# hyunlord/hnm_recommendation

Measured on AMD Instinct MI355X. Metric: recommendations/sec (batched users, K=12) at 1/2/4/8 MI355X; % HBM roofline, higher is better.
Workload: dtype f16+f32; 1 GPU; ncf: BASELINE configs[1] NeuralCF dim=64, full H&M shape, batch=4096 users/rank, K=12; users=1371980, items=105542, batch_per_rank=4096, k=12, parallelism=single, model=NeuralCF, mf_dim=64, weights=init, scan=certified f16 pre-filter + exact fp32 re-scoring (ncf_cert.hip)

## Files before the change

hnm_recommendation_amd/_lib.py:

```python
from __future__ import annotations

import ctypes as C
import os
import threading
import weakref

import torch

PKG = os.path.dirname(os.path.abspath(__file__))
LIB_PATH = os.environ.get("HNM_LIB_PATH") or os.path.join(PKG, "libhnm_mi355x.so")

HNM_OK, HNM_EINVAL, HNM_EOOB, HNM_EHIP, HNM_ENOMEM, HNM_EUNSUPPORTED, HNM_ECOLL = 0, -1, -2, -3, -4, -5, -6

_p = C.c_void_p
_i64 = C.c_int64
_i32 = C.c_int32
_f32 = C.c_float


class NcfWeights(C.Structure):
    _fields_ = [("gmf_user", _p), ("gmf_item", _p), ("mlp_user", _p), ("mlp_item", _p),
                ("w1", _p), ("b1", _p), ("w2", _p), ("b2", _p), ("wp", _p), ("bp", _p),
                ("num_users", _i64), ("num_items", _i64), ("mf", _i32), ("h0", _i32),
                ("h1", _i32), ("h2", _i32), ("item_proj", _p)]
# ... 258 lines not shown


def abort_pending(device):
    check(fn("hnm_ctx_abort_pending")(ctx(device)), "hnm_ctx_abort_pending")


def sync_check(device):
    check(fn("hnm_ctx_check")(ctx(device)), "hnm_ctx_check")


TIME_SCORE, TIME_SPMM = 1, 2


def enable_timing(device, on=True):
    check(fn("hnm_ctx_enable_timing")(ctx(device), int(on)), "hnm_ctx_enable_timing")


def kernel_timing(device):
    t = C.c_double()
    n = _i64()
    check(fn("hnm_ctx_timing")(ctx(device), C.byref(t), C.byref(n)), "hnm_ctx_timing")
    return t.value, n.value


HNM_OPT_PREFILTER = 1
HNM_OPT_STATS = 3
HNM_OPT_STRIDED = 4
HNM_OPT_DEEP_MFMA = 5
HNM_OPT_LINEAR_MFMA = 6
HNM_OPT_NCF_TABLES = 7
HNM_OPT_SCAN_SHAPE = 8
HNM_OPT_SCAN_PIPE = 9
HNM_OPT_SCAN_SPARSE = 10


def set_option(device, option, value):
    idx = _dev_index(device)
    ctx(device)
    with _lock:
        _opts.setdefault(idx, {})[int(option)] = int(value)
    for c in _device_ctxs(idx):
        check(fn("hnm_ctx_set_option")(c.handle, int(option), int(value)), "hnm_ctx_set_option")


def set_prefilter(device, on=True):
    set_option(device, HNM_OPT_PREFILTER, int(bool(on)))


def prefilter_stats(device, reset=False, extended=False):
    ctx(device)
    n = (6 if extended == "gate" else 4) if extended else 3
    tot = [0] * n
    for c in _device_ctxs(_dev_index(device)):
        out = (_i64 * n)()
        check(fn("hnm_ctx_prefilter_stats_ex")(c.handle, out, n, int(reset)),
              "hnm_ctx_prefilter_stats_ex")
        for j in range(n):
            tot[j] += int(out[j])
    return tuple(tot)


def ptr(t):
    return None if t is None else _p(t.data_ptr())
```

hnm_recommendation_amd/csrc/api.hip:

```cpp
#include <stdlib.h>
#include <string.h>

#include "hnm_device.h"
#include "hnm_internal.h"
#include "linear_mfma.h"

static thread_local char g_err[512] = "";

void hnm_set_error(const char* fmt, ...) {
  va_list ap;
  va_start(ap, fmt);
  vsnprintf(g_err, sizeof(g_err), fmt, ap);
  va_end(ap);
}

extern "C" int hnm_abi_version(void) { return HNM_ABI_VERSION; }
extern "C" const char* hnm_last_error(void) { return g_err; }

extern "C" hnm_status hnm_ctx_create(int device, hnm_ctx** out) {
  HNM_REQUIRE(out, HNM_EINVAL, "hnm_ctx_create: out is NULL");
  int ndev = 0;
  HNM_HIP_CHECK(hipGetDeviceCount(&ndev));
  HNM_REQUIRE(device >= 0 && device < ndev, HNM_EINVAL, "hnm_ctx_create: no device %d (%d visible)",
              device, ndev);
  const HnmDeviceGuard guard(device);
  hnm_ctx* c = (hnm_ctx*)calloc(1, sizeof(hnm_ctx));
  HNM_REQUIRE(c, HNM_ENOMEM, "hnm_ctx_create: out of host memory");
  c->device = device;
  c->stream = 0;
  hipDeviceProp_t prop;
  if (hipGetDeviceProperties(&prop, device) == hipSuccess) c->num_cus = prop.multiProcessorCount;
  if (c->num_cus <= 0) c->num_cus = 256;
  c->prefilter = 1;
  c->strided = 0;
  c->deep_mfma = 1;
#ifndef HNM_LINEAR_MFMA_DEFAULT
#define HNM_LINEAR_MFMA_DEFAULT 1
#endif
  c->linear_mfma = HNM_LINEAR_MFMA_DEFAULT;
  c->ncf_tables = 1;
  c->scan_shape = 1;
  c->scan_pipe = 1;
  c->scan_sparse = 1;
  if (hipMalloc((void**)&c->err_dev, 64) != hipSuccess) {
    free(c);
    hnm_set_error("hnm_ctx_create: hipMalloc of the error word failed");
    return HNM_ENOMEM;
  }
  HNM_HIP_CHECK(hipMemset(c->err_dev, 0, 64));
  HNM_HIP_CHECK(hipEventCreateWithFlags(&c->chain_ev, hipEventDisableTiming));
  HNM_HIP_CHECK(hipStreamCreateWithFlags(&c->side, hipStreamNonBlocking));
  HNM_HIP_CHECK(hipEventCreateWithFlags(&c->side_in, hipEventDisableTiming));
  HNM_HIP_CHECK(hipEventCreateWithFlags(&c->side_out, hipEventDisableTiming));
  c->stats_dev = reinterpret_cast<unsigned long long*>(reinterpret_cast<char*>(c->err_dev) + 8);
  *out = c;
  return HNM_OK;
}

extern "C" hnm_status hnm_ctx_destroy(hnm_ctx* ctx) {
  HNM_CTX_DEVICE(ctx);
  if (!ctx) return HNM_OK;
  (void)hipDeviceSynchronize();
  for (int i = 0; i < ctx->cap; ++i) {
    (void)hipEventDestroy(ctx->ev0[i]);
    (void)hipEventDestroy(ctx->ev1[i]);
  }
  free(ctx->ev0);
  free(ctx->ev1);
  hnm_rccl_release(ctx);
  if (ctx->ws) (void)hipFree(ctx->ws);
  if (ctx->err_dev) (void)hipFree(ctx->err_dev);
  (void)hipEventDestroy(ctx->chain_ev);
  (void)hipEventDestroy(ctx->side_in);
  (void)hipEventDestroy(ctx->side_out);
  (void)hipStreamDestroy(ctx->side);
  free(ctx);
// ... 18 lines not shown
  return HNM_OK;
}

extern "C" hnm_status hnm_ctx_set_option(hnm_ctx* ctx, int option, int64_t value) {
  HNM_CTX_DEVICE(ctx);
  HNM_REQUIRE(ctx, HNM_EINVAL, "ctx is NULL");
  switch (option) {
    case HNM_OPT_PREFILTER:
      ctx->prefilter = value != 0;
      return HNM_OK;
    case HNM_OPT_STATS:
      ctx->stats_on = value != 0;
      return HNM_OK;
    case HNM_OPT_STRIDED:
      ctx->strided = value != 0;
      return HNM_OK;
    case HNM_OPT_DEEP_MFMA:
      ctx->deep_mfma = value != 0;
      return HNM_OK;
    case HNM_OPT_LINEAR_MFMA:
      ctx->linear_mfma = value != 0;
      return HNM_OK;
    case HNM_OPT_NCF_TABLES:
      ctx->ncf_tables = value != 0;
      return HNM_OK;
    case HNM_OPT_SCAN_SHAPE:
      ctx->scan_shape = value != 0;
      return HNM_OK;
    case HNM_OPT_SCAN_PIPE:
      ctx->scan_pipe = value != 0;
      return HNM_OK;
    case HNM_OPT_SCAN_SPARSE:
      ctx->scan_sparse = value != 0;
      return HNM_OK;
    default:
      hnm_set_error("hnm_ctx_set_option: unknown option %d", option);
      return HNM_EINVAL;
  }
}

extern "C" hnm_status hnm_ctx_prefilter_stats(hnm_ctx* ctx, int64_t* out, int reset) {
  HNM_CTX_DEVICE(ctx);
  return hnm_ctx_prefilter_stats_ex(ctx, out, 3, reset);
}

extern "C" hnm_status hnm_ctx_prefilter_stats_ex(hnm_ctx* ctx, int64_t* out, int n, int reset) {
  HNM_CTX_DEVICE(ctx);
  HNM_REQUIRE(ctx && out, HNM_EINVAL, "ctx/out is NULL");
  HNM_REQUIRE(n >= 1 && n <= HNM_STATS_N, HNM_EINVAL, "prefilter_stats: 1 <= n <= %d", HNM_STATS_N);
  int prev = -1;
  HNM_HIP_CHECK(hipGetDevice(&prev));
  struct Restore {
    int dev;
    ~Restore() { (void)hipSetDevice(dev); }
  } restore{prev};
  HNM_HIP_CHECK(hipSetDevice(ctx->device));
  HNM_HIP_CHECK(hipDeviceSynchronize());
  unsigned long long v[HNM_STATS_N];
  HNM_HIP_CHECK(hipMemcpy(v, ctx->stats_dev, sizeof(v), hipMemcpyDeviceToHost));
  for (int i = 0; i < n; ++i) out[i] = (int64_t)v[i];
  if (reset) HNM_HIP_CHECK(hipMemset(ctx->stats_dev, 0, sizeof(v)));
  return HNM_OK;
}

extern "C" hnm_status hnm_ctx_num_cus(hnm_ctx* ctx, int* out) {
  HNM_CTX_DEVICE(ctx);
// ... 759 lines not shown
```

hnm_recommendation_amd/csrc/hnm_internal.h:

```cpp
#pragma once
#include <hip/hip_runtime.h>
#include <stdarg.h>
#include <stdint.h>
#include <stdio.h>

#include <algorithm>

#include "../../include/hnm.h"

struct hnm_ctx {
  int device;
  hipStream_t stream;
  hipEvent_t chain_ev;
  hipStream_t side;
  hipEvent_t side_in, side_out;
  void* ws;
  size_t ws_size;
  unsigned* err_dev;
  int num_cus;
  int timing;
  int nev;
  int cap;
  hipEvent_t* ev0;
  hipEvent_t* ev1;
  int prefilter;
  int strided;
  int deep_mfma;
  int linear_mfma;
  int ncf_tables;
  int scan_shape;
  int scan_pipe;
  int scan_sparse;
  void* comm;
  int comm_owned;
  unsigned long long* stats_dev;
  int stats_on;
  struct {
    int kind;
    int64_t B, I;
    int K;
    const void* ids;
    const void* items;
    int flags;
  } pend;
};
struct HnmDeviceGuard {
  int prev = -1;
  explicit HnmDeviceGuard(int device) {
    int cur = -1;
    if (device >= 0 && hipGetDevice(&cur) == hipSuccess && cur != device &&
        hipSetDevice(device) == hipSuccess)
      prev = cur;
  }
  ~HnmDeviceGuard() {
    if (prev >= 0) (void)hipSetDevice(prev);
  }
  HnmDeviceGuard(const HnmDeviceGuard&) = delete;
  HnmDeviceGuard& operator=(const HnmDeviceGuard&) = delete;
};
#define HNM_CTX_DEVICE(c) const HnmDeviceGuard hnm_device_guard_((c) ? (c)->device : -1)
#define HNM_STATS_N 6
#define HNM_PEND_NCF_CERT 1
#define HNM_PEND_NCF_EXACT 2
#define HNM_PEND_DOT_CERT 3
#define HNM_PEND_DOT_EXACT 4
// ... 108 lines not shown
```

hnm_recommendation_amd/csrc/ncf.hip:

```cpp
#include <algorithm>

#include "hnm_device.h"
#include "ncf_internal.h"

template <bool DENSE>
__global__ __launch_bounds__(256, 2) void ncf32_kernel(
    const float* __restrict__ Pu,
    const float* __restrict__ WGu,
    const float* __restrict__ Qi,
    const float* __restrict__ Gi, int64_t ldg, int mf,
    const float* __restrict__ W2, int h1, int h2, const float* __restrict__ b2,
    const float* __restrict__ wm, const float* __restrict__ bp, int64_t B, int64_t I,
    int64_t ipp, const int64_t* __restrict__ mptr, const int32_t* __restrict__ midx, int K,
    float* __restrict__ cand_v, int32_t* __restrict__ cand_i, int NP,
    float* __restrict__ dense, int64_t ldo, const int32_t* __restrict__ rows,
    const int32_t* __restrict__ nrows, int dyn_cus) {
  constexpr int KS = 32;
  constexpr int RS = 68;
  constexpr int NU = 128;
  __shared__ __attribute__((aligned(16))) float qs[TILE * RS];
  __shared__ __attribute__((aligned(16))) float gs[TILE * RS];
  __shared__ __attribute__((aligned(16))) float ps[NU * 64];
  __shared__ __attribute__((aligned(16))) float gsm[4 * 32 * 32];
  extern __shared__ __attribute__((aligned(16))) float lists[];

  const int tid = threadIdx.x, lane = tid & 63, wave = tid >> 6, h = lane >> 5, j = lane & 31;
  int64_t ublk = (int64_t)blockIdx.x * NU;
  int p = blockIdx.y;
  if (rows) B = *nrows;
  if (rows && dyn_cus > 0) {
    const int64_t nb = hnm_cdiv(B, NU);
    const Partition dp = choose_partition(I, nb, dyn_cus);
    NP = dp.np;
    ipp = dp.ipp;
    const int64_t w = blockIdx.x;
    if (w >= nb * NP) return;
    ublk = w / NP * NU;
    p = (int)(w % NP);
  }
  if (ublk >= B || p >= NP) return;
  auto R = [&](int64_t b) -> int64_t { return rows ? (int64_t)rows[b] : b; };
  const int64_t u0 = ublk + wave * 32;
  const int nu = (int)std::max<int64_t>(0, std::min<int64_t>(32, B - u0));
  const int64_t part_start = (int64_t)p * ipp;
  const int64_t part_end = std::min<int64_t>(I, part_start + ipp);
  float* lv_s = lists + wave * 32 * K;
  int* li_s = reinterpret_cast<int*>(lists + 4 * 32 * K) + wave * 32 * K;

  for (int e = tid; e < NU * 16; e += 256) {
// ... 148 lines not shown
          if ((bits >> j) & 1u) score = -__builtin_inff();
        }
        if (DENSE) {
          if (ivalid) dense[(u0 + u) * ldo + item] = score;
        } else {
          const float thv = hnm_readlane_f(tvv, u);
          const int thi = hnm_readlane_i(tvi, u);
          uint64_t m = __ballot(ivalid && (score > thv || (score == thv && (int)item < thi)));
          if (m) {
            float lv = lane < K ? lv_s[u * K + lane] : -__builtin_inff();
            int li = lane < K ? li_s[u * K + lane] : HNM_SENTINEL_IDX;
            while (m) {
              const int l = __builtin_ctzll(m);
              m &= m - 1;
              list1_insert(lv, li, hnm_readlane_f(score, l), (int)base + l, K);
            }
            if (lane < K) { lv_s[u * K + lane] = lv; li_s[u * K + lane] = li; }
            const float nv = hnm_readlane_f(lv, K - 1);
            const int ni = hnm_readlane_i(li, K - 1);
            if (lane == u) { tvv = nv; tvi = ni; }
          }
        }
      }
    }
  }
  if (!DENSE) {
    for (int e = lane; e < nu * K; e += 64) {
      const int u = e / K, s = e % K;
      const int64_t o = ((u0 + u) * NP + p) * K + s;
      cand_v[o] = lv_s[e];
      cand_i[o] = li_s[e] == HNM_SENTINEL_IDX ? -1 : li_s[e];
    }
  }
}

template <int WU, int H1P, int MFH, bool DENSE>
__global__ __launch_bounds__(256, 2) void ncf_generic_kernel(
    const float* __restrict__ Pu,
    const float* __restrict__ WGu,
    const float* __restrict__ Qi,
    const float* __restrict__ Gi, int64_t ldg,
    const float* __restrict__ W2, int h1, int h2, const float* __restrict__ b2,
    const float* __restrict__ wm, const float* __restrict__ bp, int64_t B, int64_t I,
    int64_t ipp, const int64_t* __restrict__ mptr, const int32_t* __restrict__ midx, int K,
    float* __restrict__ cand_v, int32_t* __restrict__ cand_i, int NP,
    float* __restrict__ dense, int64_t ldo) {
  constexpr int KS = H1P / 2;
  constexpr int GW = 2 * MFH;
  constexpr int QRS = H1P + 4;
  constexpr int GRS = GW + 4;
  constexpr int NU = 4 * WU;
  constexpr int QF4 = TILE * H1P / 4 / 256;
  constexpr int GF4 = TILE * GW / 4 / 256;
  static_assert(QF4 >= 1 && GF4 >= 1, "tile too small");
  __shared__ __attribute__((aligned(16))) float qs[2][TILE * QRS];
  __shared__ __attribute__((aligned(16))) float gs[2][TILE * GRS];
  __shared__ __attribute__((aligned(16))) float ps[NU * H1P];
  __shared__ __attribute__((aligned(16))) float ws[NU * GW];
  __shared__ __attribute__((aligned(16))) float2 bw[32];

  const int tid = threadIdx.x;
  const int lane = tid & 63;
  const int wave = tid >> 6;
  const int h = lane >> 5;
  const int j = lane & 31;
  const int64_t ublk = (int64_t)blockIdx.x * NU;
// ... 262 lines not shown
  return HNM_OK;
}

template <bool DENSE>
static void launch_ncf32(hnm_ctx* ctx, dim3 grid, const NcfTabs& t, const hnm_ncf_weights* w,
                         int64_t B, int64_t ipp, const int64_t* mptr, const int32_t* midx, int K,
                         float* cv, int32_t* ci, int NP, float* dense, int64_t ldo,
                         const int32_t* rows = nullptr, const int32_t* nrows = nullptr,
                         int dyn_cus = 0) {
  const size_t lds = DENSE ? 0 : (size_t)4 * 32 * K * 8;
  hipLaunchKernelGGL((ncf32_kernel<DENSE>), grid, dim3(256), lds, ctx->stream, t.Pu, t.WGu, t.Qi,
                     t.G, t.ldg, w->mf, w->w2, w->h1, w->h2, w->b2, w->wp + w->mf, w->bp, B,
                     w->num_items, ipp, mptr, midx, K, cv, ci, NP, dense, ldo, rows, nrows,
                     dyn_cus);
}

template <int WU, int H1P, int MFH, bool DENSE>
static void launch_ncf(hnm_ctx* ctx, dim3 grid, const NcfTabs& t, const hnm_ncf_weights* w,
                       int64_t B, int64_t ipp, const int64_t* mptr, const int32_t* midx, int K,
                       float* cv, int32_t* ci, int NP, float* dense, int64_t ldo) {
  hipLaunchKernelGGL((ncf_generic_kernel<WU, H1P, MFH, DENSE>), grid, dim3(256), 0, ctx->stream,
                     t.Pu, t.WGu, t.Qi, t.G, t.ldg, w->w2, w->h1, w->h2, w->b2, w->wp + w->mf,
                     w->bp, B, w->num_items, ipp, mptr, midx, K, cv, ci, NP, dense, ldo);
}

size_t ncf_list_bytes(int64_t B, int64_t I, int K, int num_cus) {
  const Partition part = choose_partition(I, hnm_cdiv(B, 128), num_cus);
  const int64_t slots = std::max<int64_t>(B * part.np, list_rows_slots(B, I, num_cus));
  return hnm_align((size_t)slots * K * 4);
}

hnm_status ncf_list_rows(hnm_ctx* ctx, const hnm_ncf_weights* w, const NcfTabs& t, int64_t B,
                         const int64_t* mptr, const int32_t* midx, int K, const int32_t* rows,
                         const int32_t* nrows, float* cv, int32_t* ci, float* ov, int64_t* oi) {
  const int64_t grid = list_rows_grid(B, w->num_items, ctx->num_cus);
  launch_ncf32<false>(ctx, dim3((unsigned)grid, 1), t, w, B, 0, mptr, midx, K, cv, ci, 1, nullptr,
                      0, rows, nrows, ctx->num_cus);
  HNM_LAUNCH_CHECK();
  return hnm_topk_merge_rows(ctx, cv, ci, B, 1, 0, K, K, K, ov, oi, rows, nrows, w->num_items,
                             ctx->num_cus);
}

struct NcfCall {
  NcfTabs t;
  bool big;
  void* extra;
};

struct NcfCertUse {
  int K;
  bool strided;
};

static hnm_status ncf_tables(hnm_ctx* ctx, const hnm_ncf_weights* w, const int64_t* ids,
                             int64_t B, size_t extra, NcfCall* out, bool fill = true,
                             const NcfCertUse* cert = nullptr) {
  const bool big = w->h1 > 64 || w->mf > 64;
  const int H1P = big ? 128 : 64, GW = big ? 128 : 64;
  const int64_t I = w->num_items;
  const bool gcopy = (big ? w->mf != GW : w->mf % 4 != 0) || ((uintptr_t)w->gmf_item % 16 != 0);
  const bool qcache = w->item_proj != nullptr;
  const size_t szP = hnm_align((size_t)B * H1P * 4), szW = hnm_align((size_t)B * GW * 4);
  const size_t szQ = qcache ? 0 : hnm_align((size_t)I * H1P * 4);
  const size_t szG = gcopy ? hnm_align((size_t)I * GW * 4) : 0;
  void* wsp = ctx->ws;
  hnm_status st = HNM_OK;
  if (fill) {
    st = hnm_workspace(ctx, szP + szW + szQ + szG + extra, &wsp);
// ... 307 lines not shown
```

hnm_recommendation_amd/csrc/ncf_cert.hip:

```cpp
#include <algorithm>

#include "ncf_cert_internal.h"
#include "sample_kth.h"

namespace {

__device__ __forceinline__ float cert_row_bound(const CertParams* prm, float unit,
                                                const float* Au, int64_t b) {
  return unit * (prm->rho * (prm->c0 + Au[b]) + prm->absb);
}
__device__ __forceinline__ float cert_lower_bound(const CertParams* prm, float unit, float kv,
                                                  float e, const float* bp) {
  float l = (kv - e) / unit + bp[0];
  l -= fabsf(l) * 4.76837158203125e-07f;
  return (!prm->bad && __builtin_isfinite(l) && __builtin_isfinite(e)) ? l : -__builtin_inff();
}

__device__ __forceinline__ void cert_threshold(const CertParams* prm, float unit, const float* Au,
                                               const float* Cu, int64_t b, float l, float e,
                                               const float* bp, float* tau, int* flag) {
  const float scale = unit * (prm->c0 + Au[b] + prm->Bmax + Cu[b] * prm->Dmax);
  float tv = (l - bp[0]) * unit - e - 3.814697265625e-06f * scale;
  tv -= fabsf(tv) * 9.5367431640625e-07f;
  const bool ok = !prm->bad && __builtin_isfinite(tv) && __builtin_isfinite(scale);
// ... 345 lines not shown
  auto take = [&](size_t bytes) {
    char* p = base ? base + off : nullptr;
    off += hnm_align(bytes);
    return p;
  };
  CertWs x;
  x.prm = (CertParams*)take(sizeof(CertParams));
  x.Au = (float*)take(B * 4);
  x.Cu = (float*)take(B * 4);
  x.Cs = (float*)take(B * 4);
  x.Bs = (float*)take(I * 4);
  x.part = (float*)take(4 * 4 * (1024 + 256));
  x.Bi = (float*)take(I * 4);
  x.Di = (float*)take(I * 4);
  x.tau = (float*)take(B * 4);
  x.Eu = (float*)take(B * 4);
  x.b2s = (float*)take(32 * 4);
  x.kthv = (float*)take((size_t)B * K * 4);
  x.lb = (float*)take((size_t)B * 4);
  x.pdense = (float*)take((size_t)CERT_PROXY_USERS * I * 4);
  x.cdense = (float*)take((size_t)B * sh.nch * 4);
  x.sidx = (int32_t*)take((size_t)sh.nch * 4);
  x.sloo = strided ? (int32_t*)take((size_t)CERT_PROXY_USERS * sh.nch * 4) : nullptr;
  x.sidx2 = strided ? (int32_t*)take((size_t)sh.ns * 4) : nullptr;
  x.sdense = strided ? (float*)take((size_t)B * sh.ns * 4) : nullptr;
  x.kth2 = strided ? (float*)take((size_t)B * K * 4) : nullptr;
  x.gate = (int*)take(4);
  x.gcnt = (unsigned long long*)take(4 * 8);
  x.kthi = (int64_t*)take((size_t)B * K * 8);
  x.cnt = (int*)take((size_t)B * sh.part.np * 4);
  x.flag = (int*)take(B * 4);
  x.ovf_cnt = (int32_t*)take(256);
  x.ovf_rows = (int32_t*)take(B * 4);
  x.buf = (int32_t*)take((size_t)B * sh.part.np * sh.capp * 4);
  x.bufd = (float*)take((size_t)B * sh.part.np * sh.capp * 4);
  x.P16 = (_Float16*)take((size_t)B * 64 * 2);
  x.WG16 = (_Float16*)take((size_t)B * 64 * 2);
  x.Q16 = (_Float16*)take((size_t)I * 64 * 2);
  x.G16 = (_Float16*)take((size_t)I * 64 * 2);
  x.W2h = (_Float16*)take(32 * 64 * 2);
  x.wmh = (_Float16*)take(32 * 2);
  x.W3h = (_Float16*)take(16 * 32 * 2);
  x.wph = (_Float16*)take(16 * 2);
  x.b3s = (float*)take(16 * 4);
  x.u = (float*)take(32 * 4);
  const size_t lb = ncf_list_bytes(B, I, K, num_cus);
  x.cv = (float*)take(lb);
  x.ci = (int32_t*)take(lb);
  if (w) *w = x;
  return off;
}

ScanArgs scan_args(const CertWs& x, int64_t B, bool deep) {
  ScanArgs a{};
  a.W3h = deep ? x.W3h : nullptr;
  a.wph = x.wph;
  a.b3s = x.b3s;
  a.P16 = x.P16;
  a.WG16 = x.WG16;
  a.Q16 = x.Q16;
  a.G16 = x.G16;
  a.W2h = x.W2h;
  a.wmh = x.wmh;
  a.b2s = x.b2s;
  a.Bi = x.Bs;
  a.Di = x.Di;
// ... 119 lines not shown
  const CertPlan pl = cert_plan(ctx, B, I, K, scratch, strided);
  const CertShape& sh = pl.sh;
  const CertWs& x = pl.ws;
  const int64_t ublocks = hnm_cdiv(B, 128);
  if (lb != nullptr || strided) {
    hipLaunchKernelGGL(cert_tau_kernel, dim3((unsigned)hnm_cdiv(B, 256)), dim3(256), 0,
                       ctx->stream, lb ? lb : x.lb, x.Au, x.Cu, x.Eu, x.prm, w->bp, B, x.tau,
                       x.flag);
    HNM_LAUNCH_CHECK();
  }
  ScanArgs a = scan_args(x, B, dp != nullptr);
  a.I = I;
  a.mptr = mptr;
  a.midx = midx;
  a.tau = x.tau;
  a.cnt = x.cnt;
  a.buf = x.buf;
  a.segd = x.bufd;
  a.capp = sh.capp;
  a.ipp = sh.part.ipp;
  a.NP = sh.part.np;
  hnm_timer_begin(ctx, HNM_TIME_SCORE);
  cert_launch_scan(ctx, SCAN_THRESH, dim3((unsigned)sh.part.np, (unsigned)ublocks), a);
  hnm_timer_end(ctx, HNM_TIME_SCORE);
  HNM_LAUNCH_CHECK();
  cert_launch_rescore(ctx, w, t, B, pl, K, short_ok, ov, oi, dp);
  HNM_LAUNCH_CHECK();
  if (dp) {
    *ovf_rows = x.ovf_rows;
    *ovf_cnt = x.ovf_cnt;
    return HNM_OK;
  }
  hnm_status st =
      ncf_list_rows(ctx, w, t, B, mptr, midx, K, x.ovf_rows, x.ovf_cnt, x.cv, x.ci, ov, oi);
  if (st || !short_ok) return st;
  return hnm_topk_trim_below(ctx, ov, oi, B, K, lb);
}

hnm_status ncf_cert_topk(hnm_ctx* ctx, const hnm_ncf_weights* w, const NcfTabs& t, int64_t B,
                         const int64_t* mptr, const int32_t* midx, int K, void* scratch,
                         bool strided, float* ov, int64_t* oi) {
  hnm_status st = ncf_cert_begin(ctx, w, t, B, mptr, midx, K, scratch, strided, nullptr);
  if (st) return st;
  return ncf_cert_finish(ctx, w, t, B, mptr, midx, K, scratch, strided, nullptr, 0, ov, oi);
}

hnm_status ncf_deep_cert_topk(hnm_ctx* ctx, const hnm_ncf_weights* w, const CertDeep& dp,
                              const NcfTabs& t, int64_t B, const int64_t* mptr,
                              const int32_t* midx, int K, void* scratch, float* ov, int64_t* oi,
                              int32_t** ovf_rows, int32_t** ovf_cnt, bool* pruned) {
  hnm_status st = ncf_cert_begin(ctx, w, t, B, mptr, midx, K, scratch, false, nullptr, nullptr, &dp);
  if (st) return st;
  const int64_t I = w->num_items;
  const CertPlan pl = cert_plan(ctx, B, I, K, scratch, false);
  const CertShape& sh = pl.sh;
  const CertWs& x = pl.ws;
  const int np_rows = (int)std::min<int64_t>(CERT_PROXY_USERS, B);
  HNM_HIP_CHECK(hipMemsetAsync(x.gcnt, 0, 8, ctx->stream));
  hipLaunchKernelGGL(cert_predict_kernel,
                     dim3((unsigned)std::min<int64_t>(64, hnm_cdiv(I, 256)), (unsigned)np_rows),
                     dim3(256), 0, ctx->stream, x.pdense, I, K, x.kthv, x.Eu, x.Bs, x.Cs, x.Di,
                     x.prm, x.gcnt);
  HNM_LAUNCH_CHECK();
  unsigned long long pc = 0;
  HNM_HIP_CHECK(hipMemcpyAsync(&pc, x.gcnt, 8, hipMemcpyDeviceToHost, ctx->stream));
  HNM_HIP_CHECK(hipStreamSynchronize(ctx->stream));
  const int64_t limit = std::min<int64_t>(I / 16, (int64_t)sh.part.np * sh.capp / 2);
// ... 33 lines not shown
```

hnm_recommendation_amd/csrc/ncf_cert_internal.h:

```cpp
#pragma once
#include "hnm_device.h"
#include "ncf_internal.h"

constexpr int64_t CERT_MIN_ITEMS = 8192;
constexpr float CERT_RHO = 0.0029296875f;
constexpr float CERT_RHO_DEEP = 0.00390625f;
constexpr int CERT_MAX_NP = 64;
constexpr int CERT_PROXY_USERS = 8;
#ifndef CERT_CHAMPIONS_AB
#define CERT_CHAMPIONS_AB 2048
#endif
constexpr int64_t CERT_CHAMPIONS = CERT_CHAMPIONS_AB;
constexpr int64_t CERT_GROUP_MIN = 48;
constexpr int CERT_STRIDE = 8;
constexpr int64_t CERT_GATE_GAIN = 150;
#define HNM_SCAN_OCC 3
constexpr int CERT_WG_PER_CU = HNM_SCAN_OCC;

enum { CM_P, CM_Q, CM_WG, CM_G, CM_B, CM_D, CM_N };

struct CertParams {
  unsigned mx[CM_N];
  float s1, sw, sm, sgu, sgi;
  float s3;
  float unit, cg;
  float rho;
  float c0, absb, Bmax, Dmax;
  int bad;
};

__device__ __forceinline__ int korig(int t) { return 2 * (t & 31) + (t >> 5); }

struct CertWs {
  CertParams* prm;
  float *Au, *Cu, *Bi, *Di, *tau, *Eu, *b2s, *kthv, *lb, *pdense, *cdense, *part;
  float *Bs, *Cs;
  int32_t* sidx;
  int32_t* sloo;
  int32_t* sidx2;
  float* sdense;
  float* kth2;
  int* gate;
  unsigned long long* gcnt;
  int64_t* kthi;
  int *cnt, *flag;
  int32_t *buf, *ovf_cnt, *ovf_rows;
  float* bufd;
  _Float16 *P16, *WG16, *Q16, *G16, *W2h, *wmh;
  _Float16 *W3h, *wph;
  float *b3s, *u;
  float* cv;
  int32_t* ci;
};

struct CertShape {
  int64_t nch, gsz;
  int64_t ns;
  Partition part;
  int capp;
};

struct StatBlocks {
  int items, users;
};

enum { SCAN_SAMPLE = 0, SCAN_THRESH = 1, SCAN_DEBUG = 2 };

struct ScanArgs {
  const _Float16* P16;
  const _Float16* WG16;
  const _Float16* Q16;
  const _Float16* G16;
  const _Float16* W2h;
  const _Float16* wmh;
  const float* b2s;
  const _Float16* W3h;
  const _Float16* wph;
  const float* b3s;
  const float* Bi;
  const float* Di;
  const float* Cu;
  const float* Eu;
  const CertParams* prm;
  int64_t B;
  int64_t I;
// ... 33 lines not shown
```

hnm_recommendation_amd/csrc/ncf_cert_params.hip:

```cpp
#include <algorithm>

#include "ncf_cert_internal.h"
#include "linear_mfma.h"

namespace {


__device__ __forceinline__ float cert_vk(const float* W2, int h1, int h2, const float* wm, int k) {
  float v = 0.f;
  for (int j = 0; j < h2; ++j) v += fabsf(wm[j]) * fabsf(W2[j * h1 + k]);
  return v;
}

__device__ __forceinline__ void cert_fill_vs(float* vs, const float* __restrict__ W2, int h1,
                                             int h2, const float* __restrict__ wm) {
  const int tid = threadIdx.x;
  if (tid < 64) {
    const int k = korig(tid);
    vs[tid] = k < h1 ? cert_vk(W2, h1, h2, wm, k) : 0.f;
  }
}

__device__ __forceinline__ float cert_sum8(const float (&v8)[8], int lane) {
  const bool b5 = lane & 32, b4 = lane & 16, b3 = lane & 8;
// ... 225 lines not shown
#pragma unroll
      for (int r = 0; r < 16; ++r) {
        const int64_t b = t0 + r0 + r;
        if (b < B) {
          const int64_t id = a.ids[b];
          const bool ok = id >= 0 && id < a.num_users;
          if (!ok && lane == 0) hnm_flag(err, HNM_ERR_OOB);
          const float wg = ncf_gather_scale(a.gmf_user, id, a.mf, a.mf, a.wp, kc, ok);
          const float pv = stage[(r0 + r) * 64 + lane];
          a.Pu[b * 64 + lane] = pv;
          a.WGu[b * 64 + lane] = wg;
          cert_user_stats(vt, fabsf(pv), wg, b, lane, Au, Cu, m0, m1);
        }
      }
      __syncthreads();
    }
  }
  cert_block_maxima(m0, m1, m2, m3, red, part, items ? blk : item_blocks + blk);
}

__device__ __forceinline__ float pow2_below_inv(float m) {
  int e;
  (void)frexpf(m, &e);
  return ldexpf(1.f, -e);
}

__global__ __launch_bounds__(256) void cert_scales_kernel(const float* __restrict__ W2, int h1,
                                                          int h2, const float* __restrict__ b2,
                                                          const float* __restrict__ wm,
                                                          const float* __restrict__ bp,
                                                          CertParams* prm,
                                                          const float* __restrict__ part,
                                                          int item_blocks, int user_blocks,
                                                          int* __restrict__ ovf_cnt, CertDeep dp) {
  __shared__ float red[7][4];
  __shared__ float pm[4][6];
  const int tid = threadIdx.x, lane = tid & 63, wave = tid >> 6;
  {
    float q = 0.f, g = 0.f, bb = 0.f, dd = 0.f, pp = 0.f, wg = 0.f;
    const int nblk = item_blocks + user_blocks;
    for (int b0 = 0; b0 < nblk; b0 += 8 * 256) {
      float4 v[8];
#pragma unroll
      for (int k = 0; k < 8; ++k)
        v[k] = *reinterpret_cast<const float4*>(part + 4 * std::min(b0 + 256 * k + tid, nblk - 1));
#pragma unroll
      for (int k = 0; k < 8; ++k) {
        const int blk = b0 + 256 * k + tid;
        if (blk < item_blocks) {
          q = nmax(q, v[k].x); g = nmax(g, v[k].y); bb = nmax(bb, v[k].z); dd = nmax(dd, v[k].w);
        } else if (blk < nblk) {
          pp = nmax(pp, v[k].x); wg = nmax(wg, v[k].y);
        }
      }
    }
    q = wave_max(q); g = wave_max(g); bb = wave_max(bb); dd = wave_max(dd);
    pp = wave_max(pp); wg = wave_max(wg);
    if (lane == 0) {
      pm[wave][0] = q; pm[wave][1] = g; pm[wave][2] = bb; pm[wave][3] = dd;
      pm[wave][4] = pp; pm[wave][5] = wg;
    }
    __syncthreads();
    if (tid < 6) {
      float m = pm[0][tid];
      for (int w = 1; w < 4; ++w) m = nmax(m, pm[w][tid]);
      const int slot = tid == 0 ? CM_Q : tid == 1 ? CM_G : tid == 2 ? CM_B : tid == 3 ? CM_D
                     : tid == 4 ? CM_P : CM_WG;
      prm->mx[slot] = __float_as_uint(m);
    }
    if (tid == 0 && ovf_cnt) *ovf_cnt = 0;
    __syncthreads();
  }
  float mW = 0.f, vsum = 0.f, mwm = 0.f, mb2 = 0.f, c0 = 0.f, swm = 0.f;
  for (int e = tid; e < h2 * h1; e += 256) {
    const float w = fabsf(W2[e]);
    mW = nmax(mW, w);
    vsum += fabsf(wm[e / h1]) * w;
  }
  float mrow = 0.f;
  for (int j0 = 0; j0 < h2; j0 += 32) {
    const int j = j0 + (tid >> 3);
    float rs = 0.f;
    if (j < h2)
      for (int k = tid & 7; k < h1; k += 8) rs += fabsf(W2[j * h1 + k]);
    rs += __shfl_xor(rs, 1);
    rs += __shfl_xor(rs, 2);
    rs += __shfl_xor(rs, 4);
    mrow = nmax(mrow, rs);
  }
  for (int j = tid; j < h2; j += 256) {
    mwm = nmax(mwm, fabsf(wm[j]));
    mb2 = nmax(mb2, fabsf(b2[j]));
    c0 += fabsf(wm[j]) * fabsf(b2[j]);
    swm += fabsf(wm[j]);
  }
  mW = wave_max(mW);
  mrow = wave_max(mrow);
  mwm = wave_max(mwm);
  mb2 = wave_max(mb2);
  vsum = wave_sum(vsum);
  c0 = wave_sum(c0);
  swm = wave_sum(swm);
  if (lane == 0) {
// ... 156 lines not shown
  if (l >= 32) return;
  float v = 0.f;
  if (l < h2)
    for (int m = 0; m < dp.h3; ++m) v += fabsf(dp.wp3[m]) * fabsf(dp.W3[m * h2 + l]);
  u[l] = v;
}

StatBlocks cert_stat_blocks(int64_t B, int64_t I, bool fused) {
  const int rows = fused ? 64 : 4;
  return {(int)std::min<int64_t>(1024, hnm_cdiv(I, rows)),
          (int)std::min<int64_t>(256, hnm_cdiv(B, rows))};
}

}

hnm_status cert_prepare(hnm_ctx* ctx, const hnm_ncf_weights* w, const NcfTabs& t, int64_t B,
                        const CertWs& x, const CertDeep* dp) {
  const int64_t I = w->num_items;
  const StatBlocks sb = cert_stat_blocks(B, I, t.stats);
  const int ib = sb.items, ub = sb.users;
  const float* wm = w->wp + w->mf;
  const CertDeep dv = dp ? *dp : CertDeep{};
  if (dp) {
    hipLaunchKernelGGL(cert_deep_u_kernel, dim3(1), dim3(64), 0, ctx->stream, dv, w->h2, x.u);
    HNM_LAUNCH_CHECK();
    wm = x.u;
  }
  if (!t.stats) {
    hipLaunchKernelGGL(cert_stats_kernel, dim3(ib + ub), dim3(256), 0, ctx->stream, t, B, I, w->mf,
                       w->w2, w->h1, w->h2, wm, x.prm, x.Au, x.Cu, x.Bi, x.Di, x.part, ib, ub);
    HNM_LAUNCH_CHECK();
  }
  hipLaunchKernelGGL(cert_scales_kernel, dim3(1), dim3(256), 0, ctx->stream, w->w2, w->h1, w->h2,
                     w->b2, wm, w->bp, x.prm, x.part, ib, ub, x.ovf_cnt, dv);
  HNM_LAUNCH_CHECK();
  const int cb = (int)std::min<int64_t>(2048, std::max<int64_t>(1, hnm_cdiv(I * 16, 256)));
  hipLaunchKernelGGL(cert_convert_kernel, dim3(cb), dim3(256), 0, ctx->stream, t, B, I, w->mf,
                     x.prm, x.P16, x.WG16, x.Q16, x.G16, w->w2, w->h1, w->h2, w->b2, wm, x.W2h,
                     x.wmh, x.b2s, x.Bi, x.Cu, x.Bs, x.Cs, dv, x.W3h, x.wph, x.b3s);
  HNM_LAUNCH_CHECK();
  return HNM_OK;
}

hnm_status ncf_cert_tables(hnm_ctx* ctx, const hnm_ncf_weights* w, const int64_t* ids, int64_t B,
                           float* Pu, float* WGu, float* Qi, int K, void* scratch, bool strided) {
  const int64_t I = w->num_items;
  const CertWs x = cert_plan(ctx, B, I, K, scratch, strided).ws;
  const StatBlocks sb = cert_stat_blocks(B, I, true);
  const NcfTablesArgs a{w->mlp_user, w->mlp_item, w->gmf_user, w->w1,  w->b1, w->wp,
                        w->item_proj, ids,         w->num_users, w->h0, w->h1, w->mf,
                        Pu,           WGu,         Qi,           w->gmf_item, w->mf};
  hipLaunchKernelGGL(ncf_tables_kernel, dim3(sb.items + sb.users), dim3(256), 0, ctx->stream, a, B,
                     I, w->w2, w->h2, w->wp + w->mf, x.Au, x.Cu, x.Bi, x.Di, x.part, sb.items,
                     sb.users, ctx->err_dev);
  HNM_LAUNCH_CHECK();
  return HNM_OK;
}
```

hnm_recommendation_amd/csrc/ncf_internal.h:

```cpp
#pragma once
#include "hnm_internal.h"

struct NcfTabs {
  const float* Pu;
  const float* WGu;
  const float* Qi;
  const float* G;
  int64_t ldg;
  bool stats;
};

__device__ __forceinline__ float ncf_gather_scale(const float* __restrict__ tab, int64_t id,
                                                  int ld, int d, const float* __restrict__ s,
                                                  int c, bool ok) {
  return (ok && c < d) ? tab[id * ld + c] * s[c] : 0.f;
}

hnm_status ncf_list_rows(hnm_ctx* ctx, const hnm_ncf_weights* w, const NcfTabs& t, int64_t B,
                         const int64_t* mptr, const int32_t* midx, int K, const int32_t* rows,
                         const int32_t* nrows, float* cv, int32_t* ci, float* ov, int64_t* oi);
size_t ncf_list_bytes(int64_t B, int64_t I, int K, int num_cus);

struct CertDeep {
  const float* W3;
  const float* b3;
  const float* wp3;
  int h3;
  const float* gmf_user;
  const float* gmf_item;
  const float* wp;
  const int64_t* ids;
};

bool ncf_deep_cert_eligible(const hnm_ncf_deep_weights* dw, int K);
hnm_status ncf_deep_cert(hnm_ctx* ctx, const hnm_ncf_deep_weights* dw, const int64_t* ids,
                         int64_t B, const int64_t* mptr, const int32_t* midx, int K, float* ov,
                         int64_t* oi, int32_t** ovf_rows, int32_t** ovf_cnt, bool* pruned);
hnm_status ncf_deep_cert_debug(hnm_ctx* ctx, const hnm_ncf_deep_weights* dw, const int64_t* ids,
                               int64_t B, float* approx, int64_t lda, float* bound);

bool ncf_cert_eligible(const hnm_ncf_weights* w, int K);
size_t ncf_cert_bytes(const hnm_ctx* ctx, int64_t B, int64_t I, int K, bool strided);
hnm_status ncf_cert_tables(hnm_ctx* ctx, const hnm_ncf_weights* w, const int64_t* ids, int64_t B,
                           float* Pu, float* WGu, float* Qi, int K, void* scratch, bool strided);
hnm_status ncf_cert_topk(hnm_ctx* ctx, const hnm_ncf_weights* w, const NcfTabs& t, int64_t B,
                         const int64_t* mptr, const int32_t* midx, int K, void* scratch,
                         bool strided, float* ov, int64_t* oi);
hnm_status ncf_cert_begin(hnm_ctx* ctx, const hnm_ncf_weights* w, const NcfTabs& t, int64_t B,
                          const int64_t* mptr, const int32_t* midx, int K, void* scratch,
                          bool strided, float* lb, float* lists = nullptr,
                          const CertDeep* dp = nullptr);
hnm_status ncf_cert_finish(hnm_ctx* ctx, const hnm_ncf_weights* w, const NcfTabs& t, int64_t B,
                           const int64_t* mptr, const int32_t* midx, int K, void* scratch,
// ... 11 lines not shown
```

include/hnm.h:

```cpp
#ifndef HNM_H_
#define HNM_H_

#include <stddef.h>
#include <stdint.h>

#ifdef __cplusplus
extern "C" {
#endif

#define HNM_ABI_VERSION 1

typedef int32_t hnm_status;
enum {
  HNM_OK = 0,
  HNM_EINVAL = -1,
  HNM_EOOB = -2,
  HNM_EHIP = -3,
  HNM_ENOMEM = -4,
  HNM_EUNSUPPORTED = -5,
  HNM_ECOLL = -6
};

typedef struct hnm_ctx hnm_ctx;
typedef struct hnm_spmm_plan hnm_spmm_plan;

int hnm_abi_version(void);
const char* hnm_last_error(void);

hnm_status hnm_ctx_create(int device, hnm_ctx** out);
hnm_status hnm_ctx_destroy(hnm_ctx* ctx);
hnm_status hnm_ctx_set_stream(hnm_ctx* ctx, void* hip_stream);
hnm_status hnm_ctx_reserve(hnm_ctx* ctx, size_t bytes);
hnm_status hnm_ctx_check(hnm_ctx* ctx);
hnm_status hnm_ctx_num_cus(hnm_ctx* ctx, int* out);
hnm_status hnm_ctx_abort_pending(hnm_ctx* ctx);
enum { HNM_OPT_PREFILTER = 1,
       HNM_OPT_STATS = 3,
       HNM_OPT_STRIDED = 4,
       HNM_OPT_DEEP_MFMA = 5   ,
       HNM_OPT_LINEAR_MFMA = 6  };
#define HNM_OPT_NCF_TABLES 7
#define HNM_OPT_SCAN_SHAPE 8
#define HNM_OPT_SCAN_PIPE 9
#define HNM_OPT_SCAN_SPARSE 10
hnm_status hnm_ctx_set_option(hnm_ctx* ctx, int option, int64_t value);
hnm_status hnm_ctx_prefilter_stats(hnm_ctx* ctx, int64_t* out, int reset);
hnm_status hnm_ctx_prefilter_stats_ex(hnm_ctx* ctx, int64_t* out, int n, int reset);
hnm_status hnm_ctx_enable_timing(hnm_ctx* ctx, int mask);
hnm_status hnm_ctx_timing(hnm_ctx* ctx, double* total_ms, int64_t* launches);

hnm_status hnm_gather_rows_f32(hnm_ctx* ctx, const float* table, int64_t rows, int64_t ld,
                               int d, const int64_t* ids, int64_t n, float* out,
                               int64_t ldo);

hnm_status hnm_linear_rows_f32(hnm_ctx* ctx, const float* X, int64_t ldx, const int64_t* ids,
                               int64_t x_rows, int64_t M, int K, const float* W,
                               int64_t ldw, const float* bias, int N, float* Y, int64_t ldy,
                               int pair_permute);

hnm_status hnm_dot_topk_f32(hnm_ctx* ctx, const float* user_tab, int64_t num_users,
                            int64_t ldu, const int64_t* user_ids, int64_t B,
                            const float* item_tab, int64_t num_items, int64_t ldi, int d,
                            const float* user_bias, const float* item_bias,
                            const float* const_bias, const int64_t* mask_ptr,
                            const int32_t* mask_idx, int k, float* out_val,
                            int64_t* out_idx);
hnm_status hnm_dot_topk_begin_f32(hnm_ctx* ctx, const float* user_tab, int64_t num_users,
                                  int64_t ldu, const int64_t* user_ids, int64_t B,
                                  const float* item_tab, int64_t num_items, int64_t ldi, int d,
                                  const float* user_bias, const float* item_bias,
                                  const float* const_bias, const int64_t* mask_ptr,
                                  const int32_t* mask_idx, int k, float* lower_bound);
hnm_status hnm_dot_topk_begin_lists_f32(hnm_ctx* ctx, const float* user_tab, int64_t num_users,
                                        int64_t ldu, const int64_t* user_ids, int64_t B,
                                        const float* item_tab, int64_t num_items, int64_t ldi,
                                        int d, const float* user_bias, const float* item_bias,
                                        const float* const_bias, const int64_t* mask_ptr,
// ... 301 lines not shown
```

Before: 2.352 million users/s.

## Fuse NCF overflow-list candidate merge into scoring kernel via last-block tickets

Result: no change. 2.353 million users/s, median of 3 (+0.0%).

```diff
diff --git a/hnm_recommendation_amd/_lib.py b/hnm_recommendation_amd/_lib.py
--- a/hnm_recommendation_amd/_lib.py
+++ b/hnm_recommendation_amd/_lib.py
@@ -314,6 +314,7 @@
 HNM_OPT_SCAN_SHAPE = 8
 HNM_OPT_SCAN_PIPE = 9
 HNM_OPT_SCAN_SPARSE = 10
+HNM_OPT_NCF_LIST_MERGE = 11
 
 
 def set_option(device, option, value):
diff --git a/hnm_recommendation_amd/csrc/api.hip b/hnm_recommendation_amd/csrc/api.hip
--- a/hnm_recommendation_amd/csrc/api.hip
+++ b/hnm_recommendation_amd/csrc/api.hip
@@ -42,6 +42,7 @@
   c->scan_shape = 1;
   c->scan_pipe = 1;
   c->scan_sparse = 1;
+  c->ncf_list_merge = 1;
   if (hipMalloc((void**)&c->err_dev, 64) != hipSuccess) {
     free(c);
     hnm_set_error("hnm_ctx_create: hipMalloc of the error word failed");
@@ -126,6 +127,9 @@
       return HNM_OK;
     case HNM_OPT_SCAN_SPARSE:
       ctx->scan_sparse = value != 0;
+      return HNM_OK;
+    case HNM_OPT_NCF_LIST_MERGE:
+      ctx->ncf_list_merge = value != 0;
       return HNM_OK;
     default:
       hnm_set_error("hnm_ctx_set_option: unknown option %d", option);
diff --git a/hnm_recommendation_amd/csrc/hnm_internal.h b/hnm_recommendation_amd/csrc/hnm_internal.h
--- a/hnm_recommendation_amd/csrc/hnm_internal.h
+++ b/hnm_recommendation_amd/csrc/hnm_internal.h
@@ -31,6 +31,7 @@
   int scan_shape;
   int scan_pipe;
   int scan_sparse;
+  int ncf_list_merge;
   void* comm;
   int comm_owned;
   unsigned long long* stats_dev;
diff --git a/hnm_recommendation_amd/csrc/ncf.hip b/hnm_recommendation_amd/csrc/ncf.hip
--- a/hnm_recommendation_amd/csrc/ncf.hip
+++ b/hnm_recommendation_amd/csrc/ncf.hip
@@ -3,7 +3,7 @@
 #include "hnm_device.h"
 #include "ncf_internal.h"
 
-template <bool DENSE>
+template <bool DENSE, bool MERGE = false>
 __global__ __launch_bounds__(256, 2) void ncf32_kernel(
     const float* __restrict__ Pu,
     const float* __restrict__ WGu,
@@ -14,7 +14,8 @@
     int64_t ipp, const int64_t* __restrict__ mptr, const int32_t* __restrict__ midx, int K,
     float* __restrict__ cand_v, int32_t* __restrict__ cand_i, int NP,
     float* __restrict__ dense, int64_t ldo, const int32_t* __restrict__ rows,
-    const int32_t* __restrict__ nrows, int dyn_cus) {
+    const int32_t* __restrict__ nrows, int dyn_cus, int* __restrict__ tickets = nullptr,
+    float* __restrict__ out_v = nullptr, int64_t* __restrict__ out_i = nullptr) {
   constexpr int KS = 32;
   constexpr int RS = 68;
   constexpr int NU = 128;
@@ -229,6 +230,50 @@
       cand_i[o] = li_s[e] == HNM_SENTINEL_IDX ? -1 : li_s[e];
     }
   }
+  if constexpr (MERGE) {
+    __shared__ int last;
+    asm volatile("s_waitcnt vmcnt(0)" ::: "memory");
+    __syncthreads();
+    if (tid == 0) {
+      __builtin_amdgcn_fence(__ATOMIC_RELEASE, "agent");
+      asm volatile("s_waitcnt vmcnt(0)" ::: "memory");
+      last = atomicAdd(&tickets[ublk / NU], 1) == NP - 1;
+    }
+    __syncthreads();
+    if (!last) return;
+    __builtin_amdgcn_fence(__ATOMIC_ACQUIRE, "agent");
+    asm volatile("s_waitcnt vmcnt(0)" ::: "memory");
+    __syncthreads();
+    const float* cv = cand_v;
+    const int32_t* ci = cand_i;
+    const int64_t n = (int64_t)NP * K;
+    for (int64_t b = ublk + wave; b < std::min<int64_t>(B, ublk + NU); b += 4) {
+      WaveTopK<1> M;
+      M.init();
+      constexpr int U = 4;
+      for (int64_t base = 0; base < n; base += 64 * U) {
+        int32_t ii[U];
+        float vv[U];
+#pragma unroll
+        for (int u = 0; u < U; ++u) {
+          const int64_t q = base + 64 * u + lane;
+          ii[u] = -1;
+          vv[u] = -__builtin_inff();
+          if (q < n) {
+            ii[u] = ci[b * n + q];
+            vv[u] = cv[b * n + q];
+          }
+        }
+#pragma unroll
+        for (int u = 0; u < U; ++u) {
+          const bool ok = ii[u] >= 0;
+          M.offer(ok ? vv[u] : -__builtin_inff(), ok ? (int)ii[u] : HNM_SENTINEL_IDX, ok, K);
+        }
+      }
+      const int64_t ob = R(b);
+      M.store(out_v ? out_v + ob * K : nullptr, out_i + ob * K, K);
+    }
+  }
 }
 
 template <int WU, int H1P, int MFH, bool DENSE>
@@ -557,8 +602,17 @@
 
 hnm_status ncf_list_rows(hnm_ctx* ctx, const hnm_ncf_weights* w, const NcfTabs& t, int64_t B,
                          const int64_t* mptr, const int32_t* midx, int K, const int32_t* rows,
-                         const int32_t* nrows, float* cv, int32_t* ci, float* ov, int64_t* oi) {
+                         const int32_t* nrows, float* cv, int32_t* ci, float* ov, int64_t* oi,
+                         int* tickets) {
   const int64_t grid = list_rows_grid(B, w->num_items, ctx->num_cus);
+  if (tickets) {
+    hipLaunchKernelGGL((ncf32_kernel<false, true>), dim3((unsigned)grid, 1), dim3(256),
+                       (size_t)4 * 32 * K * 8, ctx->stream, t.Pu, t.WGu, t.Qi, t.G, t.ldg, w->mf,
+                       w->w2, w->h1, w->h2, w->b2, w->wp + w->mf, w->bp, B, w->num_items, 0, mptr,
+                       midx, K, cv, ci, 1, nullptr, 0, rows, nrows, ctx->num_cus, tickets, ov, oi);
+    HNM_LAUNCH_CHECK();
+    return HNM_OK;
+  }
   launch_ncf32<false>(ctx, dim3((unsigned)grid, 1), t, w, B, 0, mptr, midx, K, cv, ci, 1, nullptr,
                       0, rows, nrows, ctx->num_cus);
   HNM_LAUNCH_CHECK();
diff --git a/hnm_recommendation_amd/csrc/ncf_cert.hip b/hnm_recommendation_amd/csrc/ncf_cert.hip
--- a/hnm_recommendation_amd/csrc/ncf_cert.hip
+++ b/hnm_recommendation_amd/csrc/ncf_cert.hip
@@ -401,6 +401,7 @@
   x.flag = (int*)take(B * 4);
   x.ovf_cnt = (int32_t*)take(256);
   x.ovf_rows = (int32_t*)take(B * 4);
+  x.ltick = (int*)take((size_t)hnm_cdiv(B, 128) * 4);
   x.buf = (int32_t*)take((size_t)B * sh.part.np * sh.capp * 4);
   x.bufd = (float*)take((size_t)B * sh.part.np * sh.capp * 4);
   x.P16 = (_Float16*)take((size_t)B * 64 * 2);
@@ -586,7 +587,8 @@
     return HNM_OK;
   }
   hnm_status st =
-      ncf_list_rows(ctx, w, t, B, mptr, midx, K, x.ovf_rows, x.ovf_cnt, x.cv, x.ci, ov, oi);
+      ncf_list_rows(ctx, w, t, B, mptr, midx, K, x.ovf_rows, x.ovf_cnt, x.cv, x.ci, ov, oi,
+                    ctx->ncf_list_merge ? x.ltick : nullptr);
   if (st || !short_ok) return st;
   return hnm_topk_trim_below(ctx, ov, oi, B, K, lb);
 }
diff --git a/hnm_recommendation_amd/csrc/ncf_cert_internal.h b/hnm_recommendation_amd/csrc/ncf_cert_internal.h
--- a/hnm_recommendation_amd/csrc/ncf_cert_internal.h
+++ b/hnm_recommendation_amd/csrc/ncf_cert_internal.h
@@ -51,6 +51,7 @@
   float *b3s, *u;
   float* cv;
   int32_t* ci;
+  int* ltick;
 };
 
 struct CertShape {
diff --git a/hnm_recommendation_amd/csrc/ncf_cert_params.hip b/hnm_recommendation_amd/csrc/ncf_cert_params.hip
--- a/hnm_recommendation_amd/csrc/ncf_cert_params.hip
+++ b/hnm_recommendation_amd/csrc/ncf_cert_params.hip
@@ -281,7 +281,9 @@
                                                           CertParams* prm,
                                                           const float* __restrict__ part,
                                                           int item_blocks, int user_blocks,
-                                                          int* __restrict__ ovf_cnt, CertDeep dp) {
+                                                          int* __restrict__ ovf_cnt,
+                                                          int* __restrict__ ltick, int ntick,
+                                                          CertDeep dp) {
   __shared__ float red[7][4];
   __shared__ float pm[4][6];
   const int tid = threadIdx.x, lane = tid & 63, wave = tid >> 6;
@@ -318,6 +320,7 @@
       prm->mx[slot] = __float_as_uint(m);
     }
     if (tid == 0 && ovf_cnt) *ovf_cnt = 0;
+    for (int e = tid; e < ntick; e += 256) ltick[e] = 0;
     __syncthreads();
   }
   float mW = 0.f, vsum = 0.f, mwm = 0.f, mb2 = 0.f, c0 = 0.f, swm = 0.f;
@@ -540,7 +543,8 @@
     HNM_LAUNCH_CHECK();
   }
   hipLaunchKernelGGL(cert_scales_kernel, dim3(1), dim3(256), 0, ctx->stream, w->w2, w->h1, w->h2,
-                     w->b2, wm, w->bp, x.prm, x.part, ib, ub, x.ovf_cnt, dv);
+                     w->b2, wm, w->bp, x.prm, x.part, ib, ub, x.ovf_cnt, x.ltick,
+                     (int)hnm_cdiv(B, 128), dv);
   HNM_LAUNCH_CHECK();
   const int cb = (int)std::min<int64_t>(2048, std::max<int64_t>(1, hnm_cdiv(I * 16, 256)));
   hipLaunchKernelGGL(cert_convert_kernel, dim3(cb), dim3(256), 0, ctx->stream, t, B, I, w->mf,
diff --git a/hnm_recommendation_amd/csrc/ncf_internal.h b/hnm_recommendation_amd/csrc/ncf_internal.h
--- a/hnm_recommendation_amd/csrc/ncf_internal.h
+++ b/hnm_recommendation_amd/csrc/ncf_internal.h
@@ -18,7 +18,8 @@
 
 hnm_status ncf_list_rows(hnm_ctx* ctx, const hnm_ncf_weights* w, const NcfTabs& t, int64_t B,
                          const int64_t* mptr, const int32_t* midx, int K, const int32_t* rows,
-                         const int32_t* nrows, float* cv, int32_t* ci, float* ov, int64_t* oi);
+                         const int32_t* nrows, float* cv, int32_t* ci, float* ov, int64_t* oi,
+                         int* tickets = nullptr);
 size_t ncf_list_bytes(int64_t B, int64_t I, int K, int num_cus);
 
 struct CertDeep {
diff --git a/include/hnm.h b/include/hnm.h
--- a/include/hnm.h
+++ b/include/hnm.h
@@ -43,6 +43,7 @@
 #define HNM_OPT_SCAN_SHAPE 8
 #define HNM_OPT_SCAN_PIPE 9
 #define HNM_OPT_SCAN_SPARSE 10
+#define HNM_OPT_NCF_LIST_MERGE 11
 hnm_status hnm_ctx_set_option(hnm_ctx* ctx, int option, int64_t value);
 hnm_status hnm_ctx_prefilter_stats(hnm_ctx* ctx, int64_t* out, int reset);
 hnm_status hnm_ctx_prefilter_stats_ex(hnm_ctx* ctx, int64_t* out, int n, int reset);
```
